# stdio2016/pfann

Measured on AMD Instinct MI355X. Metric: query segments/sec, 10 s @ SNR 0 queries vs 1M-segment db (exact flat IP top-100 + sequence match), higher is better.
Workload: dtype f32

## Files before the change

### include/pfann_amd.h

```cpp
#ifndef PFANN_AMD_H
#define PFANN_AMD_H

#include <stdint.h>

#ifdef __cplusplus
extern "C" {
#endif

#define PFANN_SEQSCORE_VERSION 20220625002LL


long long version(void);

int seq_score(void *index, const int64_t *song_pos, int n_songs, const float *query,
              int query_len, const int64_t *labels, int top_k, float *song_scores,
              int frame_shift_mul, float score_alpha);

const char *pfann_last_error(void);

typedef struct pfann_ctx pfann_ctx;

typedef struct pfann_config {
    int32_t segment_len;
    int32_t stft_n;
// ... 33 lines not shown
int pfann_segment_embed_at(pfann_ctx *ctx, const float *wav_dev, const int64_t *starts_dev,
                           int64_t B, float *emb_dev, int normalize, void *stream);

int pfann_pcm16_to_mono(pfann_ctx *ctx, const int16_t *pcm_dev, int64_t n_frames, int n_ch,
                        float *wav_dev, void *stream);

int pfann_pcm16_files_to_mono(pfann_ctx *ctx, const void *const *host_pcm, const int64_t *n_samples, const int64_t *dst_off,
                              int n_files, int16_t *pcm_dev, int64_t total, float *wav_dev, void *stream);

typedef struct pfann_wav_info {
    int64_t n_frames;
    int64_t data_pos;
    int32_t n_ch;
    int32_t sample_rate;
    int32_t status;
    int32_t reserved;
} pfann_wav_info;
#define PFANN_WAV_EOPEN (-1)
#define PFANN_WAV_EFORMAT (-2)
#define PFANN_WAV_ECODEC (-3)
#define PFANN_WAV_EWIDTH (-4)
#define PFANN_WAV_EREAD (-5)
int pfann_wav_probe(const char *const *paths, int n, int n_threads, pfann_wav_info *info);
int pfann_wav_read(const char *const *paths, int n, int n_threads, pfann_wav_info *info, const int64_t *dst_off,
                   int16_t *dst, int64_t dst_cap);

int pfann_resample_to_mono(pfann_ctx *ctx, const int16_t *pcm_dev, int n_ch, const float *kernels_dev, int old_rate,
                           int new_rate, int width, const int64_t *plan_dev, int n_pieces, int64_t n_out, float *tmp_dev,
                           float *wav_dev, void *stream);

int64_t pfann_debug_activation(pfann_ctx *ctx, int idx, int64_t B, float *host, int64_t cap);
void pfann_debug_keep(pfann_ctx *ctx, int on);

int pfann_set_fused_layernorm(pfann_ctx *ctx, int on);

int pfann_set_encoder_precision(pfann_ctx *ctx, int mode);

int pfann_prewarm(int device);

int64_t pfann_set_plan_batch(pfann_ctx *ctx, int64_t n);

int pfann_set_streams(pfann_ctx *ctx, int n);

typedef struct pfann_db pfann_db;

pfann_db *pfann_db_create(int d, int device);
void pfann_db_destroy(pfann_db *db);
int pfann_db_dim(pfann_db *db);
int64_t pfann_db_ntotal(pfann_db *db);

int pfann_db_load(pfann_db *db, const float *emb, int emb_is_device, int64_t n,
                  const int64_t *song_pos_host, int n_songs, int64_t label_base);

#define PFANN_DB_F32 0
#define PFANN_DB_F16 1
int pfann_db_set_storage(pfann_db *db, int mode);

int pfann_db_set_prefilter(pfann_db *db, int on);

int pfann_search_topk(pfann_db *db, const float *q_dev, int64_t nq, int k, float *D_dev,
                      int64_t *I_dev, void *stream);

int pfann_search_bound(pfann_db *db, const float *q_dev, int64_t nq, int k, int m, float *lb_dev, void *stream);
int pfann_search_topk_bounded(pfann_db *db, const float *q_dev, int64_t nq, int k, const float *lb_dev,
                              float *D_dev, int64_t *I_dev, void *stream);

// ... 49 lines not shown
```

### pfann_amd/csrc/api.hip

```cpp
#include <math.h>
#include <stdarg.h>
#include <stdlib.h>
#include <string.h>

#include <algorithm>
#include <cmath>
#include <map>
#include <mutex>

#include "kernels.h"

namespace pfann { int launch_rows_to_half(const float *x, int64_t n, int d, void *xh, float *norm_max_dev, hipStream_t s); }

__global__ void noop_api_kernel() {}
static int launch_noop_api() {
    hipLaunchKernelGGL(noop_api_kernel, dim3(1), dim3(1), 0, 0);
    return hipGetLastError() == hipSuccess ? 0 : -1;
}

namespace pfann {

static thread_local char g_err[1024] = "";
void set_error(const char *fmt, ...) {
    va_list ap;
// ... 9 lines not shown
static hipEvent_t g_pending = nullptr;
bool prof_on() { return g_prof; }
static hipEvent_t get_event() {
    if (!g_pool.empty()) { hipEvent_t e = g_pool.back(); g_pool.pop_back(); return e; }
    hipEvent_t e;
    (void)hipEventCreate(&e);
    return e;
}
void prof_begin(const char *, hipStream_t s) {
    g_pending = get_event();
    (void)hipEventRecord(g_pending, s);
}
void prof_end(const char *tag, hipStream_t s, double work) {
    hipEvent_t e1 = get_event();
    (void)hipEventRecord(e1, s);
    g_recs.push_back({tag, g_pending, e1, work});
    g_pending = nullptr;
}

}

using namespace pfann;

struct pfann_ctx {
    pfann_config cfg;
    int device;
    MelPlan mel;
    bool mel_ready = false;
    int F, T;
    SubLayer sub[16];
    float *g_w1 = nullptr, *g_b1 = nullptr, *g_w2 = nullptr, *g_b2 = nullptr;
    std::map<std::string, bool> loaded;
    int n_expected = 0;
    float *buf[2] = {nullptr, nullptr};
    int64_t buf_elems[2] = {0, 0};
    float *mel_buf = nullptr;
    double *scratch = nullptr;
    std::vector<float> w1_host, b1_host;
    float gram[14] = {};
    bool gram_ready = false;
    bool fused = false;
    int precision = 0;
    int64_t plan_batch = 0;
    int n_streams = 1;
    hipStream_t side[8] = {};
    hipEvent_t ev_fork = nullptr, ev_join[8] = {};
    float *part[2] = {nullptr, nullptr};
    float *splitk = nullptr;
    size_t splitk_bytes = 0;
    float *stats = nullptr;
    int64_t part_slots = 0;
    bool keep = false;
    int64_t keep_B = 0;
    float *dbg[16] = {};
    float *dbg_tmp = nullptr;
    int64_t dbg_cap = 0;
};

extern "C" int pfann_set_streams(pfann_ctx *c, int n);

static int build_plan(pfann_ctx *c) {
    const pfann_config &g = c->cfg;
    const int ch[9] = {1, g.d, g.d, 2 * g.d, 2 * g.d, 4 * g.d, 4 * g.d, g.h, g.h};
    int F = c->F, T = c->T;
    for (int i = 0; i < 8; ++i) {
        const int st = g.stride_t[i] > 0 ? g.stride_t[i] : 2;
        const int sf = g.stride_f[i] > 0 ? g.stride_f[i] : 2;
        const int p1 = (T - 1) / st * st + 3 - T, p2 = (F - 1) / sf * sf + 3 - F;
        const int T1 = (T - 1) / st + 1, F2 = (F - 1) / sf + 1;
// ... 34 lines not shown
    if (c->cfg.max_batch <= 0) c->cfg.max_batch = 512;
    const int n_fft = cfg->stft_n;
    int log2n = 0;
    while ((1 << log2n) < n_fft) ++log2n;
    if ((1 << log2n) != n_fft || n_fft < 64 || n_fft > 4096) { set_error("stft_n must be a power of two in 64..4096"); delete c; return nullptr; }
    if (cfg->n_mels % 1 != 0 || cfg->n_mels <= 0) { set_error("bad n_mels"); delete c; return nullptr; }
    MelPlan &m = c->mel;
    memset(&m, 0, sizeof(m));
    m.seg_len = cfg->segment_len; m.n_fft = n_fft; m.hop = cfg->stft_hop; m.n_mels = cfg->n_mels;
    m.n_frames = 1 + cfg->segment_len / cfg->stft_hop;
    m.n_freqs = n_fft / 2 + 1; m.log2n = log2n;
    m.power = cfg->power; m.pad_reflect = cfg->pad_reflect; m.log_mode = cfg->log_mode;
    m.spec_norm_max = cfg->spec_norm_max; m.log_eps = cfg->log_eps;
    if (m.pad_reflect && n_fft / 2 >= cfg->segment_len) { set_error("reflect padding needs stft_n/2 < segment_len"); delete c; return nullptr; }
    std::vector<float> win(n_fft);
    std::vector<float2> tw(n_fft / 2);
    for (int n = 0; n < n_fft; ++n) win[n] = (float)(0.5 - 0.5 * cos(2.0 * M_PI * n / n_fft));
    for (int j = 0; j < n_fft / 2; ++j) {
        tw[j].x = (float)cos(-2.0 * M_PI * j / n_fft);
        tw[j].y = (float)sin(-2.0 * M_PI * j / n_fft);
    }
    if (hipMalloc(&m.window, n_fft * sizeof(float)) != hipSuccess ||
        hipMalloc(&m.twiddle, (n_fft / 2) * sizeof(float2)) != hipSuccess) { set_error("hipMalloc failed"); delete c; return nullptr; }
    (void)hipMemcpy(m.window, win.data(), n_fft * sizeof(float), hipMemcpyHostToDevice);
    (void)hipMemcpy(m.twiddle, tw.data(), (n_fft / 2) * sizeof(float2), hipMemcpyHostToDevice);
    c->F = cfg->n_mels;
    c->T = m.n_frames;
    if (build_plan(c)) { delete c; return nullptr; }
    c->n_expected = 8 * 8 + 4;
    for (int i = 0; i < 16; ++i) {
        const int64_t e = (int64_t)c->sub[i].co * c->sub[i].Fo * c->sub[i].To;
        c->buf_elems[i & 1] = std::max(c->buf_elems[i & 1], e);
    }
    c->fused = fused_supported(c->sub, 16) && getenv("PFANN_NO_FUSE") == nullptr;
    if (!c->fused && cfg->fuller && getenv("PFANN_NO_FUSE") == nullptr)
        fprintf(stderr, "pfann_amd: this model's layer shapes (an Fo*To that is not a power of two, or channel counts not "
                        "multiples of 4) are outside the LayerNorm-fused GEMM path; using the separate-LayerNorm kernels\n");
    if (getenv("PFANN_STREAMS")) pfann_set_streams(c, atoi(getenv("PFANN_STREAMS")));
    for (int i = 0; i < 16; ++i) {
        const SubLayer &L = c->sub[i];
        const int rps = L.Fo * L.To;
        const int64_t slots = (int64_t)(rps >= 64 ? rps / 64 : 1) * cdiv(L.co, 64);
        c->part_slots = std::max(c->part_slots, slots);
    }
    if (hipMalloc(&c->scratch, 16 * sizeof(double)) != hipSuccess) {
        set_error("hipMalloc failed");
        delete c;
        return nullptr;
    }
    return c;
}

void pfann_destroy(pfann_ctx *c) {
    if (!c) return;
    (void)hipSetDevice(c->device);
    (void)hipDeviceSynchronize();
    for (int i = 0; i < 16; ++i) {
        if (c->sub[i].w) (void)hipFree(c->sub[i].w);
        if (c->sub[i].w_hi) { (void)hipFree(c->sub[i].w_hi); (void)hipFree(c->sub[i].w_lo); }
        if (c->sub[i].w22) (void)hipFree(c->sub[i].w22);
        if (c->sub[i].bias) (void)hipFree(c->sub[i].bias);
        if (c->sub[i].ln_w) (void)hipFree(c->sub[i].ln_w);
        if (c->sub[i].ln_b) (void)hipFree(c->sub[i].ln_b);
        if (c->dbg[i]) (void)hipFree(c->dbg[i]);
    }
    float *ptrs[] = {c->g_w1, c->g_b1, c->g_w2, c->g_b2, c->buf[0], c->buf[1], c->part[0], c->part[1], c->splitk, c->stats, c->mel_buf, c->mel.window,
                     c->mel.fb_val, c->dbg_tmp};
    for (float *p : ptrs) if (p) (void)hipFree(p);
    if (c->mel.twiddle) (void)hipFree(c->mel.twiddle);
    if (c->mel.fb_ptr) (void)hipFree(c->mel.fb_ptr);
    if (c->mel.fb_idx) (void)hipFree(c->mel.fb_idx);
    if (c->scratch) (void)hipFree(c->scratch);
    delete c;
}

int pfann_set_melbank(pfann_ctx *c, const float *fb, int n_freqs, int n_mels) {
    if (n_freqs != c->mel.n_freqs || n_mels != c->mel.n_mels) {
        set_error("melbank shape [%d,%d] != [%d,%d]", n_freqs, n_mels, c->mel.n_freqs, c->mel.n_mels);
        return -3;
    }
    PF_HIP(hipSetDevice(c->device));
    std::vector<int> ptr(n_mels + 1, 0), idx;
    std::vector<float> val;
    int mx = 0;
    for (int m = 0; m < n_mels; ++m) {
        for (int k = 0; k < n_freqs; ++k) {
            const float v = fb[(size_t)k * n_mels + m];
            if (v != 0.0f) { idx.push_back(k); val.push_back(v); }
        }
        ptr[m + 1] = (int)idx.size();
        mx = std::max(mx, ptr[m + 1] - ptr[m]);
    }
    if (idx.empty()) { idx.push_back(0); val.push_back(0.f); }
    MelPlan &mp = c->mel;
    if (mp.fb_ptr) { (void)hipFree(mp.fb_ptr); (void)hipFree(mp.fb_idx); (void)hipFree(mp.fb_val); }
    PF_HIP(hipMalloc(&mp.fb_ptr, ptr.size() * sizeof(int)));
    PF_HIP(hipMalloc(&mp.fb_idx, idx.size() * sizeof(int)));
    PF_HIP(hipMalloc(&mp.fb_val, val.size() * sizeof(float)));
    PF_HIP(hipMemcpy(mp.fb_ptr, ptr.data(), ptr.size() * sizeof(int), hipMemcpyHostToDevice));
// ... 83 lines not shown
        else if (!strcmp(name, "g.linear1.bias")) { dst = &c->g_b1; want = (int64_t)g.d * g.u; }
        else if (!strcmp(name, "g.linear2.weight")) { dst = &c->g_w2; want = (int64_t)g.d * g.u; }
        else if (!strcmp(name, "g.linear2.bias")) { dst = &c->g_b2; want = g.d; }
        else { set_error("unknown tensor %s", name); return -2; }
        if (numel != want) { set_error("%s: numel %lld != %lld", name, (long long)numel, (long long)want); return -3; }
        if (upload(dst, host, numel)) return -1;
    } else {
        set_error("unknown tensor %s", name);
        return -2;
    }
    c->loaded[name] = true;
    return 0;
}

int pfann_weights_missing(pfann_ctx *c) { return c->n_expected - (int)c->loaded.size(); }

int pfann_melspec(pfann_ctx *c, const float *segs, int64_t B, int64_t seg_stride, int remove_mean, float *out,
                  void *stream) {
    PF_HIP(hipSetDevice(c->device));
    if (!c->mel_ready) { set_error("pfann_melspec: mel filterbank not set"); return -5; }
    return launch_melspec(c->mel, segs, B, seg_stride, nullptr, remove_mean, out, (hipStream_t)stream);
}

static int keep_tap(pfann_ctx *c, int idx, const float *act, int64_t B, hipStream_t s) {
    const SubLayer &L = c->sub[idx];
    const int64_t e = (int64_t)L.co * L.Fo * L.To;
    const int64_t nb = std::min<int64_t>(B, 8);
    if (!c->dbg[idx]) PF_HIP(hipMalloc(&c->dbg[idx], 8 * e * sizeof(float)));
    PF_HIP(hipMemcpyAsync(c->dbg[idx], act, nb * e * sizeof(float), hipMemcpyDeviceToDevice, s));
    c->keep_B = nb;
    return 0;
}

static int ensure_workspace(pfann_ctx *c, bool need_mel) {
    const int64_t mb = c->cfg.max_batch;
    if (!c->buf[0]) {
        const size_t need = (size_t)mb * (c->buf_elems[0] + c->buf_elems[1]) * sizeof(float);
        size_t free_b = 0, total_b = 0;
        if (hipMemGetInfo(&free_b, &total_b) == hipSuccess && free_b < need) {
            set_error("the encoder workspace for max_batch = %lld segments needs %.1f GB but only %.1f GB of device memory are "
                      "free: lower max_batch (the tools: PFANN_MAX_BATCH)", (long long)mb, need / 1e9, free_b / 1e9);
            return -1;
        }
        PF_HIP(hipMalloc(&c->buf[0], mb * c->buf_elems[0] * sizeof(float)));
        PF_HIP(hipMalloc(&c->buf[1], mb * c->buf_elems[1] * sizeof(float)));
        PF_HIP(hipMalloc(&c->part[0], mb * c->part_slots * 2 * sizeof(float)));
        PF_HIP(hipMalloc(&c->part[1], mb * c->part_slots * 2 * sizeof(float)));
        PF_HIP(hipMalloc(&c->stats, mb * 2 * sizeof(float)));
    }
    if (need_mel && !c->mel_buf) PF_HIP(hipMalloc(&c->mel_buf, mb * (int64_t)c->F * c->T * sizeof(float)));
    return 0;
}

static int keep_tap_fused(pfann_ctx *c, int idx, const float *z, const float *part, int P, int64_t B, hipStream_t s) {
    const SubLayer &L = c->sub[idx];
    const int64_t e = (int64_t)L.co * L.Fo * L.To;
    const int64_t nb = std::min<int64_t>(B, 8);
    if (!c->dbg[idx]) PF_HIP(hipMalloc(&c->dbg[idx], 8 * e * sizeof(float)));
    c->keep_B = nb;
    return launch_ln_apply(L, z, part, P, c->dbg[idx], nb, c->cfg.activation, c->cfg.relu_after_bn, s);
}

static void build_gram(pfann_ctx *c) {
    const int co = c->sub[0].co;
    const std::vector<float> &w = c->w1_host, &b = c->b1_host;
    double Bsum = 0, Ws[3] = {0, 0, 0}, bb = 0, h[3] = {0, 0, 0}, G[3][3] = {};
    for (int o = 0; o < co; ++o) {
        Bsum += b[o];
        bb += (double)b[o] * b[o];
        for (int t = 0; t < 3; ++t) {
            Ws[t] += w[t * co + o];
            h[t] += (double)b[o] * w[t * co + o];
            for (int u = 0; u < 3; ++u) G[t][u] += (double)w[t * co + o] * w[u * co + o];
        }
    }
    const double v[14] = {Bsum, Ws[0], Ws[1], Ws[2], bb, h[0], h[1], h[2], G[0][0], G[0][1], G[0][2], G[1][1], G[1][2], G[2][2]};
    for (int i = 0; i < 14; ++i) c->gram[i] = (float)v[i];
    c->gram_ready = true;
}

static int encode_chunk_fused(pfann_ctx *c, const float *mel, int64_t B, float *emb, int normalize, hipStream_t s,
                              int64_t slot0) {
    const pfann_config &g = c->cfg;
    float *buf[2] = {c->buf[0] + slot0 * c->buf_elems[0], c->buf[1] + slot0 * c->buf_elems[1]};
    float *part[2] = {c->part[0] + slot0 * c->part_slots * 2, c->part[1] + slot0 * c->part_slots * 2};
    const bool fold_first = !c->keep && c->sub[1].axis == 1 && c->sub[0].co <= 256 &&
                            getenv("PFANN_NO_FOLD_FIRST") == nullptr;
    const int64_t Bp = c->plan_batch > 0 ? c->plan_batch : B;
    {
        size_t need = 0;
        for (int i = 1; i < 16; ++i) {
            const size_t n_i = splitk_scratch_need(c->sub[i], B, Bp);
            if (n_i <= ((size_t)256 << 20)) need = std::max(need, n_i);
        }
        if (need > c->splitk_bytes) {
            if (c->splitk) { PF_HIP(hipStreamSynchronize(s)); (void)hipFree(c->splitk); }
            c->splitk = nullptr; c->splitk_bytes = 0;
            if (hipMalloc(&c->splitk, need) == hipSuccess) c->splitk_bytes = need;
            else { c->splitk = nullptr; (void)hipGetLastError(); }
        }
    }
    if (fold_first && g.relu_after_bn && (int)c->w1_host.size() == 3 * c->sub[0].co && (int)c->b1_host.size() == c->sub[0].co) {
        if (!c->gram_ready) build_gram(c);
        if (launch_conv_first_gram_stats(c->sub[0], mel, part[0], B, c->gram, s)) return -1;
    } else if (launch_conv_first_stats(c->sub[0], mel, fold_first ? nullptr : buf[0], part[0], B, g.activation, g.relu_after_bn, s)) {
        return -1;
    }
    int P = fused_out_slots(c->sub[0], Bp);
    if (c->keep && keep_tap_fused(c, 0, buf[0], part[0], P, B, s)) return -1;
    int stats_final = 0;
    for (int i = 1; i < 16; ++i) {
        const bool first = fold_first && i == 1;
        if (c->sub[i].depthwise) {
            stats_final = 0;
            if (launch_conv_dw_ln(c->sub[i], c->sub[i - 1], first ? mel : buf[(i - 1) & 1], part[(i - 1) & 1], P, c->stats + slot0 * 2,
                                  buf[i & 1], part[i & 1], B, g.activation, g.relu_after_bn, first ? &c->sub[0] : nullptr, s)) return -1;
        } else if (launch_conv_gemm_ln(c->sub[i], c->sub[i - 1], first ? mel : buf[(i - 1) & 1], part[(i - 1) & 1], P, c->stats + slot0 * 2, buf[i & 1],
                                part[i & 1], B, g.activation, g.relu_after_bn, first ? &c->sub[0] : nullptr, c->precision, s,
                                c->n_streams == 1 || B < 128 ? c->splitk : nullptr, c->splitk_bytes, &stats_final, Bp)) return -1;
        P = fused_out_slots(c->sub[i], Bp);
        if (c->keep && keep_tap_fused(c, i, buf[i & 1], part[i & 1], P, B, s)) return -1;
    }
    return launch_myg_ln(c->sub[15], buf[1], part[1], P, g.activation, g.relu_after_bn, c->g_w1, c->g_b1,
                         c->g_w2, c->g_b2, g.d, g.u, g.h / g.d, B, emb, normalize, s, Bp);
}

static int encode_chunk1(pfann_ctx *c, const float *mel, int64_t B, float *emb, int normalize, hipStream_t s,
                         int64_t slot0) {
    if (c->fused) return encode_chunk_fused(c, mel, B, emb, normalize, s, slot0);
    const float *x = mel;
    for (int i = 0; i < 16; ++i) {
        const SubLayer &L = c->sub[i];
        float *y = c->buf[i & 1] + slot0 * c->buf_elems[i & 1];
        int rc;
        if (L.ci == 1 && !L.depthwise) rc = launch_conv_first(L, x, y, B, s);
        else if (L.depthwise) rc = launch_conv_depthwise(L, x, y, B, s);
        else rc = launch_conv_gemm(L, x, y, B, s);
        if (rc) return rc;
        if (launch_ln_act(L, y, B, c->cfg.activation, c->cfg.relu_after_bn, s)) return -1;
        if (c->keep && keep_tap(c, i, y, B, s)) return -1;
        x = y;
    }
    const pfann_config &g = c->cfg;
    return launch_myg(x, c->g_w1, c->g_b1, c->g_w2, c->g_b2, g.d, g.u, g.h / g.d, B, emb, normalize, s);
}

static int encode_chunk(pfann_ctx *c, const float *mel, int64_t B, float *emb, int normalize, hipStream_t s) {
    const int ns = (int)std::min<int64_t>(c->n_streams, B / 128);
    if (ns <= 1) return encode_chunk1(c, mel, B, emb, normalize, s, 0);
    if (!c->ev_fork) {
        PF_HIP(hipEventCreateWithFlags(&c->ev_fork, hipEventDisableTiming));
        for (int k = 0; k < 8; ++k) {
            PF_HIP(hipStreamCreateWithFlags(&c->side[k], hipStreamNonBlocking));
            PF_HIP(hipEventCreateWithFlags(&c->ev_join[k], hipEventDisableTiming));
        }
    }
    PF_HIP(hipEventRecord(c->ev_fork, s));
    const int64_t per = (int64_t)c->F * c->T;
    int64_t b0 = 0;
    for (int k = 0; k < ns; ++k) {
        const int64_t nb = B / ns + (k < B % ns ? 1 : 0);
        PF_HIP(hipStreamWaitEvent(c->side[k], c->ev_fork, 0));
        if (encode_chunk1(c, mel + b0 * per, nb, emb + b0 * c->cfg.d, normalize, c->side[k], b0)) return -1;
        PF_HIP(hipEventRecord(c->ev_join[k], c->side[k]));
        PF_HIP(hipStreamWaitEvent(s, c->ev_join[k], 0));
        b0 += nb;
    }
    return 0;
}

int pfann_encode(pfann_ctx *c, const float *mel, int64_t B, float *emb, int normalize, void *stream) {
    PF_HIP(hipSetDevice(c->device));
    if (pfann_weights_missing(c) != 0) { set_error("pfann_encode: %d state_dict tensors not loaded", pfann_weights_missing(c)); return -5; }
    hipStream_t s = (hipStream_t)stream;
    if (ensure_workspace(c, false)) return -1;
    const int64_t per = (int64_t)c->F * c->T;
    for (int64_t b0 = 0; b0 < B; b0 += c->cfg.max_batch) {
        const int64_t nb = std::min<int64_t>(c->cfg.max_batch, B - b0);
        if (encode_chunk(c, mel + b0 * per, nb, emb + b0 * c->cfg.d, normalize, s)) return -1;
    }
    return 0;
}

static int segment_embed_impl(pfann_ctx *c, const float *wav, int64_t B, int64_t seg_stride, const int64_t *starts,
                              float *emb, int normalize, void *stream) {
    PF_HIP(hipSetDevice(c->device));
    if (!c->mel_ready) { set_error("pfann_segment_embed: mel filterbank not set"); return -5; }
    if (pfann_weights_missing(c) != 0) { set_error("pfann_segment_embed: %d state_dict tensors not loaded", pfann_weights_missing(c)); return -5; }
    hipStream_t s = (hipStream_t)stream;
    if (ensure_workspace(c, true)) return -1;
    for (int64_t b0 = 0; b0 < B; b0 += c->cfg.max_batch) {
        const int64_t nb = std::min<int64_t>(c->cfg.max_batch, B - b0);
        const float *src = starts ? wav : wav + b0 * seg_stride;
        if (launch_melspec(c->mel, src, nb, seg_stride, starts ? starts + b0 : nullptr, 1, c->mel_buf, s)) return -1;
        if (encode_chunk(c, c->mel_buf, nb, emb + b0 * c->cfg.d, normalize, s)) return -1;
    }
    return 0;
}

int pfann_segment_embed(pfann_ctx *c, const float *wav, int64_t B, int64_t seg_stride, float *emb, int normalize,
                        void *stream) {
    return segment_embed_impl(c, wav, B, seg_stride, nullptr, emb, normalize, stream);
}

int pfann_segment_embed_at(pfann_ctx *c, const float *wav, const int64_t *starts_dev, int64_t B, float *emb,
                           int normalize, void *stream) {
    return segment_embed_impl(c, wav, B, 0, starts_dev, emb, normalize, stream);
}

int pfann_resample_to_mono(pfann_ctx *c, const int16_t *pcm, int n_ch, const float *kernels, int old_rate, int new_rate, int width,
                           const int64_t *plan, int n_pieces, int64_t n_out, float *tmp, float *wav, void *stream) {
    PF_HIP(hipSetDevice(c->device));
    return launch_resample_to_mono(pcm, n_ch, kernels, old_rate, new_rate, width, plan, n_pieces, n_out, tmp, wav,
                                   reinterpret_cast<float *>(c->scratch), (hipStream_t)stream);
}

int pfann_pcm16_to_mono(pfann_ctx *c, const int16_t *pcm, int64_t n_frames, int n_ch, float *wav, void *stream) {
    PF_HIP(hipSetDevice(c->device));
    if (n_ch < 1) { set_error("n_ch < 1"); return -1; }
    return launch_pcm16_to_mono(pcm, n_frames, n_ch, wav, reinterpret_cast<float *>(c->scratch), (hipStream_t)stream);
}

int pfann_pcm16_files_to_mono(pfann_ctx *c, const void *const *host_pcm, const int64_t *n_samples, const int64_t *dst_off,
                              int n_files, int16_t *pcm_dev, int64_t total, float *wav_dev, void *stream) {
    PF_HIP(hipSetDevice(c->device));
    for (int i = 0; i < n_files; ++i) {
        if (n_samples[i] <= 0) continue;
        if (dst_off[i] < 0 || dst_off[i] + n_samples[i] > total) { set_error("pcm16_files_to_mono: file %d outside the slab", i); return -1; }
        PF_HIP(hipMemcpyAsync(pcm_dev + dst_off[i], host_pcm[i], (size_t)n_samples[i] * sizeof(int16_t), hipMemcpyHostToDevice,
                              (hipStream_t)stream));
    }
    if (total <= 0) return 0;
    return launch_pcm16_to_mono(pcm_dev, total, 1, wav_dev, reinterpret_cast<float *>(c->scratch), (hipStream_t)stream);
}

void pfann_debug_keep(pfann_ctx *c, int on) { c->keep = on != 0; }

int pfann_prewarm(int device) {
    if (hipSetDevice(device) != hipSuccess) { set_error("pfann_prewarm: no HIP device %d", device); return -1; }
    int rc = launch_noop_api();
    rc |= prewarm_mel() | prewarm_encoder() | prewarm_encoder_fused() | prewarm_search() | prewarm_search_f16() | prewarm_rerank();
    if (hipDeviceSynchronize() != hipSuccess) rc = -1;
    return rc ? -1 : 0;
}

int64_t pfann_set_plan_batch(pfann_ctx *c, int64_t n) {
    c->plan_batch = n <= 0 ? 0 : (n < 65 ? 65 : n);
    return c->plan_batch;
}

int pfann_set_streams(pfann_ctx *c, int n) {
    c->n_streams = n < 1 ? 1 : (n > 8 ? 8 : n);
    return c->n_streams;
}

int pfann_set_encoder_precision(pfann_ctx *c, int mode) {
    c->precision = (mode == 1 && c->fused) ? 1 : 0;
    return c->precision;
}

int pfann_set_fused_layernorm(pfann_ctx *c, int on) {
    if (on && !fused_supported(c->sub, 16)) return 0;
    c->fused = on != 0;
    return c->fused ? 1 : 0;
}

int64_t pfann_debug_activation(pfann_ctx *c, int idx, int64_t B, float *host, int64_t cap) {
    if (idx < 0 || idx > 15 || !c->dbg[idx]) { set_error("no tap %d (call pfann_debug_keep(ctx,1) before encoding)", idx); return -1; }
    if (hipSetDevice(c->device) != hipSuccess) return -1;
// ... 381 lines not shown
```

### pfann_amd/engine.py

```python
import ctypes

import numpy as np
import torch

from . import lib as _l
from .config import config_from_params
from .synth import model_dims


def _mel_to_hz_tensor(m, scale):
    if scale == "htk":
        return 700.0 * (10.0 ** (m / 2595.0) - 1.0)
    import math
    logstep = math.log(6.4) / 27.0
    return torch.where(m >= 15.0, 1000.0 * torch.exp(logstep * (m - 15.0)), (200.0 / 3) * m)


def _hz_to_mel(f, scale):
    import math
    if scale == "htk":
        return 2595.0 * math.log10(1.0 + f / 700.0)
    if f >= 1000.0:
        return 15.0 + math.log(f / 1000.0) / (math.log(6.4) / 27.0)
    return f / (200.0 / 3)
# ... 130 lines not shown
        if sample_rate is not None and int(sample_rate) != int(self.params["sample_rate"]) and n:
            from . import resample
            key = resample.reduced_rates(sample_rate, self.params["sample_rate"])
            if key not in self._resample_tables:
                tab, old, new, width = resample.filter_table(*key)
                self._resample_tables[key] = (torch.from_numpy(tab).to(self.device), old, new, width)
            tab, old, new, width = self._resample_tables[key]
            plan, n_out = resample.piece_plan(n, int(sample_rate), int(self.params["sample_rate"]))
            plan_dev = _l.upload_async(plan, self.device, np.int64)
            tmp = torch.empty((n_ch, n_out), device=self.device, dtype=torch.float32)
            out = torch.empty((n_out,), device=self.device, dtype=torch.float32)
            if n_out:
                _l.check(self.lib.pfann_resample_to_mono(self.handle, p.data_ptr(), n_ch, tab.data_ptr(), old, new, width,
                                                         plan_dev.data_ptr(), plan.shape[0], n_out, tmp.data_ptr(),
                                                         out.data_ptr(), self._stream()), "pfann_resample_to_mono")
            return out
        out = torch.empty((n,), device=self.device, dtype=torch.float32)
        if n:
            _l.check(self.lib.pfann_pcm16_to_mono(self.handle, p.data_ptr(), n, n_ch, out.data_ptr(),
                                                  self._stream()), "pfann_pcm16_to_mono")
        return out

    def warmup(self, windows=512, group_hop=0):
        n = max(1, min(int(windows), int(self.cfg.max_batch)))
        wav = torch.zeros(self.seg_len + (n - 1) * 16, device=self.device, dtype=torch.float32)
        self.embed_windows(wav, np.arange(n, dtype=np.int64) * 16)
        self.pcm16_to_mono(torch.zeros((64, 1), dtype=torch.int16))
        torch.cuda.synchronize(self.device)
        if group_hop:
            samples = int(n * int(group_hop) * 1.12) + self.seg_len
            keep = [torch.empty(samples, dtype=dt, device=self.device) for dt in (torch.int16, torch.float32) for _ in range(2)]
            del keep

    def set_fused_layernorm(self, on=True):
        return bool(self.lib.pfann_set_fused_layernorm(self.handle, 1 if on else 0))

    def set_plan_batch(self, n=0):
        return int(self.lib.pfann_set_plan_batch(self.handle, int(n)))

    def set_encoder_precision(self, mode=0):
        return int(self.lib.pfann_set_encoder_precision(self.handle, int(mode)))

    def debug_keep(self, on=True):
        self.lib.pfann_debug_keep(self.handle, 1 if on else 0)

    def debug_activation(self, idx, B):
        from .synth import layer_plan
        L = layer_plan(self.params)[idx // 2]
        if idx % 2 == 0:
            shape = (L["co"], L["F"], L["T1"])
        else:
            shape = (L["co"], L["F2"], L["T1"])
        buf = np.empty((B,) + shape, dtype=np.float32)
        torch.cuda.synchronize(self.device)
        n = _l.check(self.lib.pfann_debug_activation(self.handle, idx, B, buf.ctypes.data, buf.size),
                     "pfann_debug_activation")
        return buf.reshape(-1)[:n].reshape((-1,) + shape)
```

### pfann_amd/lib.py

```python
import ctypes
import os
from ctypes import (POINTER, Structure, c_char_p, c_double, c_float, c_int, c_int16, c_int32, c_int64,
                    c_longlong, c_void_p)

HERE = os.path.dirname(os.path.abspath(__file__))
LIB_PATH = os.path.join(HERE, "libpfann_amd.so")


class PfannError(RuntimeError):
    pass


class Config(Structure):
    _fields_ = [("segment_len", c_int32), ("stft_n", c_int32), ("stft_hop", c_int32), ("n_mels", c_int32),
                ("power", c_int32), ("pad_reflect", c_int32), ("log_mode", c_int32),
                ("spec_norm_max", c_int32), ("log_eps", c_float),
                ("d", c_int32), ("h", c_int32), ("u", c_int32), ("fuller", c_int32),
                ("activation", c_int32), ("relu_after_bn", c_int32),
                ("stride_t", c_int32 * 8), ("stride_f", c_int32 * 8), ("max_batch", c_int32)]


class MatchResult(Structure):
    _fields_ = [("song", c_int32), ("offset", c_int32), ("shift", c_int32), ("n_cand", c_int32),
                ("score", c_double)]


class WavInfo(Structure):
    _fields_ = [("n_frames", c_int64), ("data_pos", c_int64), ("n_ch", c_int32), ("sample_rate", c_int32),
                ("status", c_int32), ("reserved", c_int32)]


SYMBOLS = {
    "version": (c_longlong, []),
    "seq_score": (c_int, [c_void_p, POINTER(c_int64), c_int, POINTER(c_float), c_int, POINTER(c_int64),
                          c_int, POINTER(c_float), c_int, c_float]),
    "pfann_last_error": (c_char_p, []),
    "pfann_create": (c_void_p, [POINTER(Config), c_int]),
    "pfann_destroy": (None, [c_void_p]),
    "pfann_set_melbank": (c_int, [c_void_p, c_void_p, c_int, c_int]),
    "pfann_load_weight": (c_int, [c_void_p, c_char_p, c_void_p, c_int64]),
    "pfann_weights_missing": (c_int, [c_void_p]),
    "pfann_melspec": (c_int, [c_void_p, c_void_p, c_int64, c_int64, c_int, c_void_p, c_void_p]),
    "pfann_encode": (c_int, [c_void_p, c_void_p, c_int64, c_void_p, c_int, c_void_p]),
    "pfann_segment_embed": (c_int, [c_void_p, c_void_p, c_int64, c_int64, c_void_p, c_int, c_void_p]),
    "pfann_segment_embed_at": (c_int, [c_void_p, c_void_p, c_void_p, c_int64, c_void_p, c_int, c_void_p]),
    "pfann_pcm16_to_mono": (c_int, [c_void_p, c_void_p, c_int64, c_int, c_void_p, c_void_p]),
    "pfann_pcm16_files_to_mono": (c_int, [c_void_p, POINTER(c_void_p), POINTER(c_int64), POINTER(c_int64), c_int, c_void_p, c_int64,
                                          c_void_p, c_void_p]),
    "pfann_wav_probe": (c_int, [POINTER(c_char_p), c_int, c_int, POINTER(WavInfo)]),
    "pfann_wav_read": (c_int, [POINTER(c_char_p), c_int, c_int, POINTER(WavInfo), POINTER(c_int64), c_void_p, c_int64]),
    "pfann_resample_to_mono": (c_int, [c_void_p, c_void_p, c_int, c_void_p, c_int, c_int, c_int, c_void_p, c_int, c_int64,
                                       c_void_p, c_void_p, c_void_p]),
    "pfann_debug_activation": (c_int64, [c_void_p, c_int, c_int64, c_void_p, c_int64]),
    "pfann_debug_keep": (None, [c_void_p, c_int]),
    "pfann_set_fused_layernorm": (c_int, [c_void_p, c_int]),
    "pfann_set_encoder_precision": (c_int, [c_void_p, c_int]),
    "pfann_prewarm": (c_int, [c_int]),
    "pfann_set_plan_batch": (c_int64, [c_void_p, c_int64]),
    "pfann_set_streams": (c_int, [c_void_p, c_int]),
    "pfann_db_create": (c_void_p, [c_int, c_int]),
    "pfann_db_destroy": (None, [c_void_p]),
    "pfann_db_set_prefilter": (c_int, [c_void_p, c_int]),
    "pfann_db_set_storage": (c_int, [c_void_p, c_int]),
    "pfann_db_dim": (c_int, [c_void_p]),
    "pfann_db_ntotal": (c_int64, [c_void_p]),
    "pfann_db_bytes": (c_int64, [c_void_p]),
    "pfann_db_load": (c_int, [c_void_p, c_void_p, c_int, c_int64, POINTER(c_int64), c_int, c_int64]),
    "pfann_search_topk": (c_int, [c_void_p, c_void_p, c_int64, c_int, c_void_p, c_void_p, c_void_p]),
    "pfann_search_bound": (c_int, [c_void_p, c_void_p, c_int64, c_int, c_int, c_void_p, c_void_p]),
    "pfann_search_topk_bounded": (c_int, [c_void_p, c_void_p, c_int64, c_int, c_void_p, c_void_p, c_void_p, c_void_p]),
    "pfann_topk_merge": (c_int, [c_void_p, c_void_p, c_void_p, c_int64, c_int, c_int, c_void_p, c_void_p,
                                 c_void_p]),
    "pfann_bound_reduce": (c_int, [c_void_p, c_void_p, c_int, c_int64, c_int, c_int, c_void_p, c_void_p]),
    "pfann_topk_merge_lists": (c_int, [c_void_p, c_void_p, c_void_p, c_int, c_int64, c_int, c_void_p, c_void_p, c_void_p]),
    "pfann_match": (c_int, [c_void_p, c_void_p, c_void_p, c_int, c_void_p, c_void_p, c_int64, c_int, c_int,
                            c_float, c_int, c_int, c_void_p, c_void_p, c_void_p]),
    "pfann_db_owned_songs": (c_int, [c_void_p, POINTER(c_int), POINTER(c_int)]),
    "pfann_db_set_owned_songs": (c_int, [c_void_p, c_int, c_int]),
    "pfann_song_scores_to_seconds": (c_int, [c_void_p, c_void_p, c_int64, c_int, c_double, c_int, c_void_p]),
    "pfann_match_pack": (c_int, [c_void_p, c_void_p, c_int64, c_void_p, c_void_p]),
    "pfann_match_pick": (c_int, [c_void_p, c_void_p, c_int, c_int64, c_void_p, c_void_p]),
    "pfann_prof_enable": (None, [c_int]),
    "pfann_prof_reset": (None, []),
    "pfann_prof_marker": (None, [c_void_p]),
    "pfann_prof_elapsed_ms": (c_double, [c_char_p, POINTER(c_int64)]),
    "pfann_prof_work": (c_double, [c_char_p]),
    "pfann_prof_tags": (c_int, [c_char_p, c_int]),
# ... 76 lines not shown
```

Before: 225,900.

## Merge encoder batches into wide spans for tail layers using a carved arena

The encoder workspace becomes a single arena carved into buffers, with a lean even-layer buffer when the first conv is folded. A new schedule runs the early layers over groups of windows, stores the activation at a cut layer where spatial size is small, and then runs the tail layers and head once over a whole span of many max_batch chunks. This cuts launch count and gives the small-spatial tail GEMMs larger batches. The cost is more complex buffer aliasing and splitting big layers into pieces. Mel spectrograms can also reuse the even buffer instead of a separate allocation.

```diff
diff --git a/include/pfann_amd.h b/include/pfann_amd.h
--- a/include/pfann_amd.h
+++ b/include/pfann_amd.h
@@ -89,6 +89,8 @@
 int64_t pfann_debug_activation(pfann_ctx *ctx, int idx, int64_t B, float *host, int64_t cap);
 void pfann_debug_keep(pfann_ctx *ctx, int on);
 
+int64_t pfann_workspace_bytes(pfann_ctx *ctx);
+
 int pfann_set_fused_layernorm(pfann_ctx *ctx, int on);
 
 int pfann_set_encoder_precision(pfann_ctx *ctx, int mode);
diff --git a/pfann_amd/csrc/api.hip b/pfann_amd/csrc/api.hip
--- a/pfann_amd/csrc/api.hip
+++ b/pfann_amd/csrc/api.hip
@@ -65,9 +65,20 @@
     float *g_w1 = nullptr, *g_b1 = nullptr, *g_w2 = nullptr, *g_b2 = nullptr;
     std::map<std::string, bool> loaded;
     int n_expected = 0;
+    char *arena = nullptr;
+    size_t arena_bytes = 0;
     float *buf[2] = {nullptr, nullptr};
+    int64_t buf_stride[2] = {0, 0};
     int64_t buf_elems[2] = {0, 0};
+    int64_t even_lean = 0;
+    int schedule = 2;
+    bool no_fold_first = false;
+    int cut = 16;
+    int64_t tail_elems[2] = {0, 0};
+    int64_t tail_slots = 0;
     float *mel_buf = nullptr;
+    size_t mel_bytes = 0;
+    bool chunk_lean = false;
     double *scratch = nullptr;
     std::vector<float> w1_host, b1_host;
     float gram[14] = {};
@@ -168,6 +179,20 @@
         const int64_t e = (int64_t)c->sub[i].co * c->sub[i].Fo * c->sub[i].To;
         c->buf_elems[i & 1] = std::max(c->buf_elems[i & 1], e);
     }
+    for (int i = 2; i < 16; i += 2)
+        c->even_lean = std::max(c->even_lean, (int64_t)c->sub[i].co * c->sub[i].Fo * c->sub[i].To);
+    c->cut = 16;
+    for (int i = 2; i < 16; ++i)
+        if (c->sub[i - 1].Fo * c->sub[i - 1].To <= 32) { c->cut = i; break; }
+    c->no_fold_first = getenv("PFANN_NO_FOLD_FIRST") != nullptr;
+    if (const char *e = getenv("PFANN_LAUNCH_GROUPS")) c->schedule = std::max(0, std::min(2, atoi(e)));
+    if (c->schedule < 2) c->cut = 16;
+    for (int i = c->cut; i < 16; ++i)
+        c->tail_elems[i & 1] = std::max(c->tail_elems[i & 1], (int64_t)c->sub[i].co * c->sub[i].Fo * c->sub[i].To);
+    for (int i = c->cut - 1; i < 16; ++i) {
+        const int rps = c->sub[i].Fo * c->sub[i].To;
+        c->tail_slots = std::max(c->tail_slots, (int64_t)(rps >= 64 ? rps / 64 : 1) * cdiv(c->sub[i].co, 64));
+    }
     c->fused = fused_supported(c->sub, 16) && getenv("PFANN_NO_FUSE") == nullptr;
     if (!c->fused && cfg->fuller && getenv("PFANN_NO_FUSE") == nullptr)
         fprintf(stderr, "pfann_amd: this model's layer shapes (an Fo*To that is not a power of two, or channel counts not "
@@ -200,7 +225,7 @@
         if (c->sub[i].ln_b) (void)hipFree(c->sub[i].ln_b);
         if (c->dbg[i]) (void)hipFree(c->dbg[i]);
     }
-    float *ptrs[] = {c->g_w1, c->g_b1, c->g_w2, c->g_b2, c->buf[0], c->buf[1], c->part[0], c->part[1], c->splitk, c->stats, c->mel_buf, c->mel.window,
+    float *ptrs[] = {c->g_w1, c->g_b1, c->g_w2, c->g_b2, reinterpret_cast<float *>(c->arena), c->splitk, c->mel_buf, c->mel.window,
                      c->mel.fb_val, c->dbg_tmp};
     for (float *p : ptrs) if (p) (void)hipFree(p);
     if (c->mel.twiddle) (void)hipFree(c->mel.twiddle);
@@ -350,23 +375,68 @@
     return 0;
 }
 
-static int ensure_workspace(pfann_ctx *c, bool need_mel) {
-    const int64_t mb = c->cfg.max_batch;
-    if (!c->buf[0]) {
-        const size_t need = (size_t)mb * (c->buf_elems[0] + c->buf_elems[1]) * sizeof(float);
-        size_t free_b = 0, total_b = 0;
-        if (hipMemGetInfo(&free_b, &total_b) == hipSuccess && free_b < need) {
-            set_error("the encoder workspace for max_batch = %lld segments needs %.1f GB but only %.1f GB of device memory are "
-                      "free: lower max_batch (the tools: PFANN_MAX_BATCH)", (long long)mb, need / 1e9, free_b / 1e9);
-            return -1;
-        }
-        PF_HIP(hipMalloc(&c->buf[0], mb * c->buf_elems[0] * sizeof(float)));
-        PF_HIP(hipMalloc(&c->buf[1], mb * c->buf_elems[1] * sizeof(float)));
-        PF_HIP(hipMalloc(&c->part[0], mb * c->part_slots * 2 * sizeof(float)));
-        PF_HIP(hipMalloc(&c->part[1], mb * c->part_slots * 2 * sizeof(float)));
-        PF_HIP(hipMalloc(&c->stats, mb * 2 * sizeof(float)));
-    }
-    if (need_mel && !c->mel_buf) PF_HIP(hipMalloc(&c->mel_buf, mb * (int64_t)c->F * c->T * sizeof(float)));
+static size_t budget_bytes(const pfann_ctx *c) {
+    const size_t mb = (size_t)c->cfg.max_batch;
+    return mb * ((size_t)(c->buf_elems[0] + c->buf_elems[1]) * sizeof(float) + (size_t)c->part_slots * 16 + 8);
+}
+
+static int ensure_arena(pfann_ctx *c, size_t need) {
+    if (need <= c->arena_bytes) return 0;
+    if (need > budget_bytes(c)) {
+        set_error("internal: an encoder workspace of %zu bytes would pass the %zu bytes of max_batch = %d", need,
+                  budget_bytes(c), c->cfg.max_batch);
+        return -1;
+    }
+    size_t free_b = 0, total_b = 0;
+    if (hipMemGetInfo(&free_b, &total_b) == hipSuccess && free_b < need) {
+        set_error("the encoder workspace for max_batch = %lld segments needs %.1f GB but only %.1f GB of device memory are "
+                  "free: lower max_batch (the tools: PFANN_MAX_BATCH)", (long long)c->cfg.max_batch, need / 1e9, free_b / 1e9);
+        return -1;
+    }
+    char *blk = nullptr;
+    PF_HIP(hipMalloc(&blk, need));
+    if (c->arena) {
+        if (hipDeviceSynchronize() != hipSuccess) { (void)hipFree(blk); set_error("hipDeviceSynchronize failed"); return -1; }
+        (void)hipFree(c->arena);
+    }
+    c->arena = blk;
+    c->arena_bytes = need;
+    return 0;
+}
+
+static int ensure_mel_buf(pfann_ctx *c) {
+    if (c->mel_buf) return 0;
+    const size_t n = (size_t)c->cfg.max_batch * c->F * c->T * sizeof(float);
+    PF_HIP(hipMalloc(&c->mel_buf, n));
+    c->mel_bytes = n;
+    return 0;
+}
+
+struct Carver {
+    char *p;
+    size_t off;
+    float *take(size_t bytes) { float *r = reinterpret_cast<float *>(p + off); off += bytes; return r; }
+};
+
+static bool fold_first_now(const pfann_ctx *c) {
+    return c->fused && !c->keep && c->sub[1].axis == 1 && c->sub[0].co <= 256 && !c->no_fold_first;
+}
+
+static size_t group_bytes_per_window(const pfann_ctx *c, bool lean) {
+    return (size_t)((lean ? c->even_lean : c->buf_elems[0]) + c->buf_elems[1]) * sizeof(float) + (size_t)c->part_slots * 16;
+}
+
+static int carve_chunk(pfann_ctx *c, bool lean) {
+    const size_t mb = (size_t)c->cfg.max_batch;
+    if (ensure_arena(c, mb * (group_bytes_per_window(c, lean) + 8))) return -1;
+    Carver a{c->arena, 0};
+    c->buf_stride[0] = lean ? c->even_lean : c->buf_elems[0];
+    c->buf_stride[1] = c->buf_elems[1];
+    c->buf[0] = a.take(mb * c->buf_stride[0] * sizeof(float));
+    c->buf[1] = a.take(mb * c->buf_stride[1] * sizeof(float));
+    c->part[0] = a.take(mb * c->part_slots * 8);
+    c->part[1] = a.take(mb * c->part_slots * 8);
+    c->stats = a.take(mb * 8);
     return 0;
 }
 
@@ -397,50 +467,98 @@
     c->gram_ready = true;
 }
 
+static int ensure_splitk(pfann_ctx *c, int64_t B, int64_t Bp, hipStream_t s) {
+    size_t need = 0;
+    for (int i = 1; i < 16; ++i) {
+        const size_t n_i = splitk_scratch_need(c->sub[i], B, Bp);
+        if (n_i <= ((size_t)256 << 20)) need = std::max(need, n_i);
+    }
+    if (need <= c->splitk_bytes) return 0;
+    float *blk = nullptr;
+    if (hipMalloc(&blk, need) != hipSuccess) { (void)hipGetLastError(); return 0; }
+    if (c->splitk) {
+        if (hipStreamSynchronize(s) != hipSuccess) { (void)hipFree(blk); set_error("hipStreamSynchronize failed"); return -1; }
+        (void)hipFree(c->splitk);
+    }
+    c->splitk = blk;
+    c->splitk_bytes = need;
+    return 0;
+}
+
+struct Stage {
+    float *act[16];
+    float *prt[16];
+    float *stats;
+};
+
+static int fused_layers(pfann_ctx *c, const Stage &st, const float *mel, int i0, int i1, int64_t B, int64_t Bp, int64_t piece,
+                        bool fold_first, int *stats_final, hipStream_t s) {
+    const pfann_config &g = c->cfg;
+    for (int i = i0; i < i1; ++i) {
+        const SubLayer &L = c->sub[i];
+        const int P = fused_out_slots(L, Bp);
+        if (i == 0) {
+            if (fold_first && g.relu_after_bn && (int)c->w1_host.size() == 3 * L.co && (int)c->b1_host.size() == L.co) {
+                if (!c->gram_ready) build_gram(c);
+                if (launch_conv_first_gram_stats(L, mel, st.prt[0], B, c->gram, s)) return -1;
+            } else if (launch_conv_first_stats(L, mel, fold_first ? nullptr : st.act[0], st.prt[0], B, g.activation, g.relu_after_bn, s)) {
+                return -1;
+            }
+            *stats_final = 0;
+            if (c->keep && keep_tap_fused(c, 0, st.act[0], st.prt[0], P, B, s)) return -1;
+            continue;
+        }
+        const bool first = fold_first && i == 1;
+        const SubLayer &Li = c->sub[i - 1];
+        const int Pin = fused_out_slots(Li, Bp);
+        const int64_t in_e = first ? (int64_t)c->F * c->T : (int64_t)Li.co * Li.Fo * Li.To;
+        const int64_t out_e = (int64_t)L.co * L.Fo * L.To;
+        const float *x0 = first ? mel : st.act[i - 1];
+        const bool may_split = piece <= 0 || (!L.depthwise && splitk_scratch_need(L, piece, Bp) > 0);
+        const int64_t step = piece > 0 && piece < B && may_split ? piece : B;
+        int sf_out = 0;
+        for (int64_t w0 = 0; w0 < B; w0 += step) {
+            const int64_t nb = std::min(step, B - w0);
+            const float *x = x0 + w0 * in_e;
+            const float *in_part = st.prt[i - 1] + w0 * Pin * 2;
+            float *y = st.act[i] + w0 * out_e, *out_part = st.prt[i] + w0 * P * 2, *stats = st.stats + w0 * 2;
+            if (L.depthwise) {
+                sf_out = 0;
+                if (launch_conv_dw_ln(L, Li, x, in_part, Pin, stats, y, out_part, nb, g.activation, g.relu_after_bn,
+                                      first ? &c->sub[0] : nullptr, s)) return -1;
+            } else {
+                sf_out = *stats_final;
+                if (launch_conv_gemm_ln(L, Li, x, in_part, Pin, stats, y, out_part, nb, g.activation, g.relu_after_bn,
+                                        first ? &c->sub[0] : nullptr, c->precision, s,
+                                        may_split && (c->n_streams == 1 || nb < 128) ? c->splitk : nullptr, c->splitk_bytes, &sf_out, Bp)) return -1;
+            }
+        }
+        *stats_final = sf_out;
+        if (c->keep && keep_tap_fused(c, i, st.act[i], st.prt[i], P, B, s)) return -1;
+    }
+    return 0;
+}
+
+static int fused_head(pfann_ctx *c, const Stage &st, int64_t B, int64_t Bp, float *emb, int normalize, hipStream_t s) {
+    const pfann_config &g = c->cfg;
+    return launch_myg_ln(c->sub[15], st.act[15], st.prt[15], fused_out_slots(c->sub[15], Bp), g.activation, g.relu_after_bn,
+                         c->g_w1, c->g_b1, c->g_w2, c->g_b2, g.d, g.u, g.h / g.d, B, emb, normalize, s, Bp);
+}
+
 static int encode_chunk_fused(pfann_ctx *c, const float *mel, int64_t B, float *emb, int normalize, hipStream_t s,
                               int64_t slot0) {
-    const pfann_config &g = c->cfg;
-    float *buf[2] = {c->buf[0] + slot0 * c->buf_elems[0], c->buf[1] + slot0 * c->buf_elems[1]};
-    float *part[2] = {c->part[0] + slot0 * c->part_slots * 2, c->part[1] + slot0 * c->part_slots * 2};
-    const bool fold_first = !c->keep && c->sub[1].axis == 1 && c->sub[0].co <= 256 &&
-                            getenv("PFANN_NO_FOLD_FIRST") == nullptr;
+    Stage st;
+    for (int i = 0; i < 16; ++i) {
+        st.act[i] = c->buf[i & 1] + slot0 * c->buf_stride[i & 1];
+        st.prt[i] = c->part[i & 1] + slot0 * c->part_slots * 2;
+    }
+    st.stats = c->stats + slot0 * 2;
+    const bool fold_first = c->chunk_lean;
     const int64_t Bp = c->plan_batch > 0 ? c->plan_batch : B;
-    {
-        size_t need = 0;
-        for (int i = 1; i < 16; ++i) {
-            const size_t n_i = splitk_scratch_need(c->sub[i], B, Bp);
-            if (n_i <= ((size_t)256 << 20)) need = std::max(need, n_i);
-        }
-        if (need > c->splitk_bytes) {
-            if (c->splitk) { PF_HIP(hipStreamSynchronize(s)); (void)hipFree(c->splitk); }
-            c->splitk = nullptr; c->splitk_bytes = 0;
-            if (hipMalloc(&c->splitk, need) == hipSuccess) c->splitk_bytes = need;
-            else { c->splitk = nullptr; (void)hipGetLastError(); }
-        }
-    }
-    if (fold_first && g.relu_after_bn && (int)c->w1_host.size() == 3 * c->sub[0].co && (int)c->b1_host.size() == c->sub[0].co) {
-        if (!c->gram_ready) build_gram(c);
-        if (launch_conv_first_gram_stats(c->sub[0], mel, part[0], B, c->gram, s)) return -1;
-    } else if (launch_conv_first_stats(c->sub[0], mel, fold_first ? nullptr : buf[0], part[0], B, g.activation, g.relu_after_bn, s)) {
-        return -1;
-    }
-    int P = fused_out_slots(c->sub[0], Bp);
-    if (c->keep && keep_tap_fused(c, 0, buf[0], part[0], P, B, s)) return -1;
+    if (ensure_splitk(c, B, Bp, s)) return -1;
     int stats_final = 0;
-    for (int i = 1; i < 16; ++i) {
-        const bool first = fold_first && i == 1;
-        if (c->sub[i].depthwise) {
-            stats_final = 0;
-            if (launch_conv_dw_ln(c->sub[i], c->sub[i - 1], first ? mel : buf[(i - 1) & 1], part[(i - 1) & 1], P, c->stats + slot0 * 2,
-                                  buf[i & 1], part[i & 1], B, g.activation, g.relu_after_bn, first ? &c->sub[0] : nullptr, s)) return -1;
-        } else if (launch_conv_gemm_ln(c->sub[i], c->sub[i - 1], first ? mel : buf[(i - 1) & 1], part[(i - 1) & 1], P, c->stats + slot0 * 2, buf[i & 1],
-                                part[i & 1], B, g.activation, g.relu_after_bn, first ? &c->sub[0] : nullptr, c->precision, s,
-                                c->n_streams == 1 || B < 128 ? c->splitk : nullptr, c->splitk_bytes, &stats_final, Bp)) return -1;
-        P = fused_out_slots(c->sub[i], Bp);
-        if (c->keep && keep_tap_fused(c, i, buf[i & 1], part[i & 1], P, B, s)) return -1;
-    }
-    return launch_myg_ln(c->sub[15], buf[1], part[1], P, g.activation, g.relu_after_bn, c->g_w1, c->g_b1,
-                         c->g_w2, c->g_b2, g.d, g.u, g.h / g.d, B, emb, normalize, s, Bp);
+    if (fused_layers(c, st, mel, 0, 16, B, Bp, 0, fold_first, &stats_final, s)) return -1;
+    return fused_head(c, st, B, Bp, emb, normalize, s);
 }
 
 static int encode_chunk1(pfann_ctx *c, const float *mel, int64_t B, float *emb, int normalize, hipStream_t s,
@@ -449,7 +567,7 @@
     const float *x = mel;
     for (int i = 0; i < 16; ++i) {
         const SubLayer &L = c->sub[i];
-        float *y = c->buf[i & 1] + slot0 * c->buf_elems[i & 1];
+        float *y = c->buf[i & 1] + slot0 * c->buf_stride[i & 1];
         int rc;
         if (L.ci == 1 && !L.depthwise) rc = launch_conv_first(L, x, y, B, s);
         else if (L.depthwise) rc = launch_conv_depthwise(L, x, y, B, s);
@@ -487,17 +605,119 @@
     return 0;
 }
 
+struct Windows {
+    const float *mel, *wav;
+    int64_t seg_stride;
+    const int64_t *starts;
+};
+
+static int mel_of(pfann_ctx *c, const Windows &in, int64_t w0, int64_t nb, float *out, hipStream_t s) {
+    const float *src = in.starts ? in.wav : in.wav + w0 * in.seg_stride;
+    return launch_melspec(c->mel, src, nb, in.seg_stride, in.starts ? in.starts + w0 : nullptr, 1, out, s);
+}
+
+static int encode_chunks(pfann_ctx *c, const Windows &in, int64_t w0, int64_t w1, float *emb, int normalize, hipStream_t s) {
+    if (w0 >= w1) return 0;
+    const bool lean = fold_first_now(c);
+    c->chunk_lean = lean;
+    if (carve_chunk(c, lean)) return -1;
+    const int64_t per = (int64_t)c->F * c->T;
+    float *mel_buf = nullptr;
+    if (!in.mel) {
+        if (lean && c->n_streams == 1 && c->buf_stride[0] >= per) mel_buf = c->buf[0];
+        else if (ensure_mel_buf(c)) return -1;
+        else mel_buf = c->mel_buf;
+    }
+    for (int64_t b0 = w0; b0 < w1; b0 += c->cfg.max_batch) {
+        const int64_t nb = std::min<int64_t>(c->cfg.max_batch, w1 - b0);
+        if (!in.mel && mel_of(c, in, b0, nb, mel_buf, s)) return -1;
+        if (encode_chunk(c, in.mel ? in.mel + b0 * per : mel_buf, nb, emb + b0 * c->cfg.d, normalize, s)) return -1;
+    }
+    return 0;
+}
+
+static int encode_all(pfann_ctx *c, const Windows &in, int64_t B, float *emb, int normalize, hipStream_t s) {
+    const int64_t mb = c->cfg.max_batch, per = (int64_t)c->F * c->T;
+    const int64_t Bp = c->plan_batch > 0 ? c->plan_batch : mb;
+    const int cut = c->cut;
+    bool merged = c->schedule > 0 && fold_first_now(c) && c->n_streams == 1 && B >= 2 * mb && mb > 64 &&
+                  (in.mel || c->even_lean >= per);
+    if (!merged) return encode_chunks(c, in, 0, B, emb, normalize, s);
+    int64_t span_max = 0;
+    const size_t budget = budget_bytes(c), grp_pw = group_bytes_per_window(c, true);
+    const int64_t x_e = cut < 16 ? (int64_t)c->sub[cut - 1].co * c->sub[cut - 1].Fo * c->sub[cut - 1].To : 0;
+    const size_t wide_pw = (size_t)x_e * sizeof(float) + (cut < 16 ? (size_t)c->tail_slots * 24 : 0) + 8;
+    const size_t pp_pw = (size_t)(c->tail_elems[0] + c->tail_elems[1]) * sizeof(float);
+    bool any_split = false;
+    if (merged) {
+        for (int i = 1; i < 16; ++i) any_split |= !c->sub[i].depthwise && splitk_scratch_need(c->sub[i], mb, Bp) > 0;
+        span_max = (int64_t)(budget / 4 / (wide_pw + pp_pw)) / mb * mb;
+        if (span_max < 2 * mb) merged = false;
+    }
+    if (!merged) return encode_chunks(c, in, 0, B, emb, normalize, s);
+
+    const int64_t Nw = B / mb * mb;
+    const int64_t unit = any_split ? mb : 128;
+    for (int64_t p0 = 0; p0 < Nw;) {
+        const int64_t span = std::min(span_max, Nw - p0);
+        int64_t G = (int64_t)((budget - (size_t)span * wide_pw) / grp_pw);
+        G = std::min(span, G >= unit ? G / unit * unit : G);
+        if (G < mb) G = mb;
+        const int64_t ng = (span + G - 1) / G;
+        G = std::min(G, ((span + ng - 1) / ng + unit - 1) / unit * unit);
+        const size_t grp_bytes = std::max((size_t)G * grp_pw, (size_t)span * pp_pw);
+        size_t need = grp_bytes + (size_t)span * wide_pw;
+        if (need > budget) return encode_chunks(c, in, p0, B, emb, normalize, s);
+        if (ensure_arena(c, std::max(need, (size_t)mb * (grp_pw + 8)))) return -1;
+        if (ensure_splitk(c, mb, Bp, s)) return -1;
+        Carver a{c->arena, 0};
+        float *even = a.take((size_t)G * c->even_lean * sizeof(float));
+        float *odd = a.take((size_t)G * c->buf_elems[1] * sizeof(float));
+        float *part0 = a.take((size_t)G * c->part_slots * 8), *part1 = a.take((size_t)G * c->part_slots * 8);
+        Carver t{c->arena, 0};
+        float *tail0 = t.take((size_t)span * c->tail_elems[0] * sizeof(float));
+        float *tail1 = t.take((size_t)span * c->tail_elems[1] * sizeof(float));
+        Carver w{c->arena, grp_bytes};
+        float *X = w.take((size_t)span * x_e * sizeof(float));
+        float *xpart = nullptr, *tpart[2] = {nullptr, nullptr};
+        if (cut < 16) {
+            xpart = w.take((size_t)span * c->tail_slots * 8);
+            tpart[0] = w.take((size_t)span * c->tail_slots * 8);
+            tpart[1] = w.take((size_t)span * c->tail_slots * 8);
+        }
+        float *stats = w.take((size_t)span * 8);
+        const int Px = cut < 16 ? fused_out_slots(c->sub[cut - 1], Bp) : 0;
+
+        int stats_final = 0;
+        for (int64_t g0 = 0; g0 < span; g0 += G) {
+            const int64_t nb = std::min(G, span - g0);
+            Stage st;
+            for (int i = 0; i < 16; ++i) { st.act[i] = i & 1 ? odd : even; st.prt[i] = i & 1 ? part1 : part0; }
+            if (cut < 16) { st.act[cut - 1] = X + g0 * x_e; st.prt[cut - 1] = xpart + g0 * Px * 2; }
+            st.stats = stats + g0 * 2;
+            const float *mel = in.mel ? in.mel + (p0 + g0) * per : even;
+            if (!in.mel && mel_of(c, in, p0 + g0, nb, even, s)) return -1;
+            if (fused_layers(c, st, mel, 0, cut, nb, Bp, mb, true, &stats_final, s)) return -1;
+            if (cut == 16 && fused_head(c, st, nb, Bp, emb + (p0 + g0) * c->cfg.d, normalize, s)) return -1;
+        }
+        if (cut < 16) {
+            Stage st;
+            for (int i = 0; i < 16; ++i) { st.act[i] = i & 1 ? tail1 : tail0; st.prt[i] = tpart[i & 1]; }
+            st.act[cut - 1] = X; st.prt[cut - 1] = xpart;
+            st.stats = stats;
+            if (fused_layers(c, st, nullptr, cut, 16, span, Bp, mb, true, &stats_final, s)) return -1;
+            if (fused_head(c, st, span, Bp, emb + p0 * c->cfg.d, normalize, s)) return -1;
+        }
+        p0 += span;
+    }
+    return encode_chunks(c, in, Nw, B, emb, normalize, s);
+}
+
 int pfann_encode(pfann_ctx *c, const float *mel, int64_t B, float *emb, int normalize, void *stream) {
     PF_HIP(hipSetDevice(c->device));
     if (pfann_weights_missing(c) != 0) { set_error("pfann_encode: %d state_dict tensors not loaded", pfann_weights_missing(c)); return -5; }
-    hipStream_t s = (hipStream_t)stream;
-    if (ensure_workspace(c, false)) return -1;
-    const int64_t per = (int64_t)c->F * c->T;
-    for (int64_t b0 = 0; b0 < B; b0 += c->cfg.max_batch) {
-        const int64_t nb = std::min<int64_t>(c->cfg.max_batch, B - b0);
-        if (encode_chunk(c, mel + b0 * per, nb, emb + b0 * c->cfg.d, normalize, s)) return -1;
-    }
-    return 0;
+    const Windows in{mel, nullptr, 0, nullptr};
+    return encode_all(c, in, B, emb, normalize, (hipStream_t)stream);
 }
 
 static int segment_embed_impl(pfann_ctx *c, const float *wav, int64_t B, int64_t seg_stride, const int64_t *starts,
@@ -505,15 +725,8 @@
     PF_HIP(hipSetDevice(c->device));
     if (!c->mel_ready) { set_error("pfann_segment_embed: mel filterbank not set"); return -5; }
     if (pfann_weights_missing(c) != 0) { set_error("pfann_segment_embed: %d state_dict tensors not loaded", pfann_weights_missing(c)); return -5; }
-    hipStream_t s = (hipStream_t)stream;
-    if (ensure_workspace(c, true)) return -1;
-    for (int64_t b0 = 0; b0 < B; b0 += c->cfg.max_batch) {
-        const int64_t nb = std::min<int64_t>(c->cfg.max_batch, B - b0);
-        const float *src = starts ? wav : wav + b0 * seg_stride;
-        if (launch_melspec(c->mel, src, nb, seg_stride, starts ? starts + b0 : nullptr, 1, c->mel_buf, s)) return -1;
-        if (encode_chunk(c, c->mel_buf, nb, emb + b0 * c->cfg.d, normalize, s)) return -1;
-    }
-    return 0;
+    const Windows in{nullptr, wav, seg_stride, starts};
+    return encode_all(c, in, B, emb, normalize, (hipStream_t)stream);
 }
 
 int pfann_segment_embed(pfann_ctx *c, const float *wav, int64_t B, int64_t seg_stride, float *emb, int normalize,
@@ -553,6 +766,8 @@
 }
 
 void pfann_debug_keep(pfann_ctx *c, int on) { c->keep = on != 0; }
+
+int64_t pfann_workspace_bytes(pfann_ctx *c) { return (int64_t)(c->arena_bytes + c->mel_bytes); }
 
 int pfann_prewarm(int device) {
     if (hipSetDevice(device) != hipSuccess) { set_error("pfann_prewarm: no HIP device %d", device); return -1; }
diff --git a/pfann_amd/engine.py b/pfann_amd/engine.py
--- a/pfann_amd/engine.py
+++ b/pfann_amd/engine.py
@@ -186,6 +186,9 @@
             keep = [torch.empty(samples, dtype=dt, device=self.device) for dt in (torch.int16, torch.float32) for _ in range(2)]
             del keep
 
+    def workspace_bytes(self):
+        return int(self.lib.pfann_workspace_bytes(self.handle))
+
     def set_fused_layernorm(self, on=True):
         return bool(self.lib.pfann_set_fused_layernorm(self.handle, 1 if on else 0))
 
diff --git a/pfann_amd/lib.py b/pfann_amd/lib.py
--- a/pfann_amd/lib.py
+++ b/pfann_amd/lib.py
@@ -53,6 +53,7 @@
                                        c_void_p, c_void_p, c_void_p]),
     "pfann_debug_activation": (c_int64, [c_void_p, c_int, c_int64, c_void_p, c_int64]),
     "pfann_debug_keep": (None, [c_void_p, c_int]),
+    "pfann_workspace_bytes": (c_int64, [c_void_p]),
     "pfann_set_fused_layernorm": (c_int, [c_void_p, c_int]),
     "pfann_set_encoder_precision": (c_int, [c_void_p, c_int]),
     "pfann_prewarm": (c_int, [c_int]),
```

Result: faster. 229,200, median of 6 (+1.5%).
